# EDAPINENUT/CBGBench

Hardware: NVIDIA H100
Metric: ligands/sec sampled (1000-step denoise, batch 64) (higher is better)
Workload: dtype f32

## Files before the change

cbgbench_b200/csrc/cbg_tc.cuh:

```cuda
#pragma once
#include <cuda_fp16.h>
#include "cbg_common.cuh"

namespace cbg_tc {

__device__ __forceinline__ uint32_t smem_u32(const void* p) { return (uint32_t)__cvta_generic_to_shared(p); }

__device__ __forceinline__ void mbar_init(uint32_t bar, uint32_t count) {
  asm volatile("mbarrier.init.shared::cta.b64 [%0], %1;" ::"r"(bar), "r"(count));
}
__device__ __forceinline__ void mbar_expect_tx(uint32_t bar, uint32_t bytes) {
  asm volatile("mbarrier.arrive.expect_tx.shared::cta.b64 _, [%0], %1;" ::"r"(bar), "r"(bytes) : "memory");
}
__device__ __forceinline__ void mbar_arrive(uint32_t bar) {
  asm volatile("mbarrier.arrive.shared::cta.b64 _, [%0];" ::"r"(bar) : "memory");
}
__device__ __forceinline__ uint64_t global_timer_ns() {
  uint64_t t;
  asm volatile("mov.u64 %0, %%globaltimer;" : "=l"(t));
  return t;
}
__device__ __forceinline__ uint32_t mbar_try_wait(uint32_t bar, uint32_t parity) {
  uint32_t done;
  asm volatile(
      "{\n\t.reg .pred p;\n\t"
      "mbarrier.try_wait.parity.shared::cta.b64 p, [%1], %2, %3;\n\t"
      "selp.u32 %0, 1, 0, p;\n\t}"
      : "=r"(done)
      : "r"(bar), "r"(parity), "r"(100000u)
      : "memory");
  return done;
}
__device__ __forceinline__ void mbar_wait(uint32_t bar, uint32_t parity) {
  uint32_t spins = 0;
  uint64_t t0 = 0;
  while (!mbar_try_wait(bar, parity)) {
    if ((++spins & 1023u) == 0u) {
      const uint64_t t = global_timer_ns();
      if (t0 == 0) t0 = t;
      else if (t - t0 > 2000000000ull) __trap();
    }
  }
}
__device__ __forceinline__ void fence_mbar_init() { asm volatile("fence.mbarrier_init.release.cluster;" ::: "memory"); }
__device__ __forceinline__ void fence_proxy_async() { asm volatile("fence.proxy.async.shared::cta;" ::: "memory"); }

__device__ __forceinline__ void bulk_g2s(uint32_t dst, const void* src, uint32_t bytes, uint32_t bar) {
  asm volatile("cp.async.bulk.shared::cluster.global.mbarrier::complete_tx::bytes [%0], [%1], %2, [%3];" ::"r"(dst),
               "l"(src), "r"(bytes), "r"(bar)
               : "memory");
}
__device__ __forceinline__ void cp_async16(uint32_t dst, const void* src) {
  asm volatile("cp.async.cg.shared.global [%0], [%1], 16;" ::"r"(dst), "l"(src) : "memory");
}
__device__ __forceinline__ void cp_async_arrive(uint32_t bar) {
  asm volatile("cp.async.mbarrier.arrive.noinc.shared::cta.b64 [%0];" ::"r"(bar) : "memory");
}

__device__ __forceinline__ void pdl_launch_dependents() { asm volatile("griddepcontrol.launch_dependents;" ::: "memory"); }
__device__ __forceinline__ void pdl_wait() { asm volatile("griddepcontrol.wait;" ::: "memory"); }

__device__ __forceinline__ void wgmma_fence() { asm volatile("wgmma.fence.sync.aligned;" ::: "memory"); }
__device__ __forceinline__ void wgmma_commit() { asm volatile("wgmma.commit_group.sync.aligned;" ::: "memory"); }
__device__ __forceinline__ void wgmma_wait0() { asm volatile("wgmma.wait_group.sync.aligned 0;" ::: "memory"); }
template <int N>
__device__ __forceinline__ void wgmma_settle(float (&d)[N]) {
#pragma unroll
  for (int i = 0; i < N; ++i) asm volatile("" : "+f"(d[i])::"memory");
}
__device__ __forceinline__ void warpgroup_sync(int wg) { asm volatile("bar.sync %0, 128;" ::"r"(1 + wg) : "memory"); }
__device__ __forceinline__ uint64_t smem_desc(uint32_t saddr, uint32_t lbo_bytes, uint32_t sbo_bytes) {
  return (uint64_t)((saddr & 0x3FFFFu) >> 4) | ((uint64_t)(lbo_bytes >> 4) << 16) | ((uint64_t)(sbo_bytes >> 4) << 32);
}
__device__ __forceinline__ void wgmma_f16_ss(float (&d)[64], uint64_t adesc, uint64_t bdesc, uint32_t accumulate) {
  asm volatile(
      "{\n\t.reg .pred p;\n\t"
      "setp.ne.b32 p, %66, 0;\n\t"
      "wgmma.mma_async.sync.aligned.m64n128k16.f32.f16.f16 "
      "{%0, %1, %2, %3, %4, %5, %6, %7, %8, %9, %10, %11, %12, %13, %14, %15, %16, %17, %18, %19, %20, %21, %22, %23, %24, %25, %26, %27, %28, %29, %30, %31, %32, %33, %34, %35, %36, %37, %38, %39, %40, %41, %42, %43, %44, %45, %46, %47, %48, %49, %50, %51, %52, %53, %54, %55, %56, %57, %58, %59, %60, %61, %62, %63}, "
      "%64, %65, p, 1, 1, 0, 0;\n\t}"
      : "+f"(d[0]), "+f"(d[1]), "+f"(d[2]), "+f"(d[3]), "+f"(d[4]), "+f"(d[5]), "+f"(d[6]), "+f"(d[7]),
        "+f"(d[8]), "+f"(d[9]), "+f"(d[10]), "+f"(d[11]), "+f"(d[12]), "+f"(d[13]), "+f"(d[14]), "+f"(d[15]),
        "+f"(d[16]), "+f"(d[17]), "+f"(d[18]), "+f"(d[19]), "+f"(d[20]), "+f"(d[21]), "+f"(d[22]), "+f"(d[23]),
        "+f"(d[24]), "+f"(d[25]), "+f"(d[26]), "+f"(d[27]), "+f"(d[28]), "+f"(d[29]), "+f"(d[30]), "+f"(d[31]),
        "+f"(d[32]), "+f"(d[33]), "+f"(d[34]), "+f"(d[35]), "+f"(d[36]), "+f"(d[37]), "+f"(d[38]), "+f"(d[39]),
        "+f"(d[40]), "+f"(d[41]), "+f"(d[42]), "+f"(d[43]), "+f"(d[44]), "+f"(d[45]), "+f"(d[46]), "+f"(d[47]),
        "+f"(d[48]), "+f"(d[49]), "+f"(d[50]), "+f"(d[51]), "+f"(d[52]), "+f"(d[53]), "+f"(d[54]), "+f"(d[55]),
        "+f"(d[56]), "+f"(d[57]), "+f"(d[58]), "+f"(d[59]), "+f"(d[60]), "+f"(d[61]), "+f"(d[62]), "+f"(d[63])
      : "l"(adesc), "l"(bdesc), "r"(accumulate));
}
__device__ __forceinline__ void wgmma_f16_ss_first(float (&d)[64], uint64_t adesc, uint64_t bdesc) {
  asm volatile(
      "{\n\t.reg .pred p;\n\t"
      "setp.ne.b32 p, %66, 0;\n\t"
      "wgmma.mma_async.sync.aligned.m64n128k16.f32.f16.f16 "
      "{%0, %1, %2, %3, %4, %5, %6, %7, %8, %9, %10, %11, %12, %13, %14, %15, %16, %17, %18, %19, %20, %21, %22, %23, %24, %25, %26, %27, %28, %29, %30, %31, %32, %33, %34, %35, %36, %37, %38, %39, %40, %41, %42, %43, %44, %45, %46, %47, %48, %49, %50, %51, %52, %53, %54, %55, %56, %57, %58, %59, %60, %61, %62, %63}, "
      "%64, %65, p, 1, 1, 0, 0;\n\t}"
      : "=f"(d[0]), "=f"(d[1]), "=f"(d[2]), "=f"(d[3]), "=f"(d[4]), "=f"(d[5]), "=f"(d[6]), "=f"(d[7]),
        "=f"(d[8]), "=f"(d[9]), "=f"(d[10]), "=f"(d[11]), "=f"(d[12]), "=f"(d[13]), "=f"(d[14]), "=f"(d[15]),
        "=f"(d[16]), "=f"(d[17]), "=f"(d[18]), "=f"(d[19]), "=f"(d[20]), "=f"(d[21]), "=f"(d[22]), "=f"(d[23]),
        "=f"(d[24]), "=f"(d[25]), "=f"(d[26]), "=f"(d[27]), "=f"(d[28]), "=f"(d[29]), "=f"(d[30]), "=f"(d[31]),
        "=f"(d[32]), "=f"(d[33]), "=f"(d[34]), "=f"(d[35]), "=f"(d[36]), "=f"(d[37]), "=f"(d[38]), "=f"(d[39]),
        "=f"(d[40]), "=f"(d[41]), "=f"(d[42]), "=f"(d[43]), "=f"(d[44]), "=f"(d[45]), "=f"(d[46]), "=f"(d[47]),
        "=f"(d[48]), "=f"(d[49]), "=f"(d[50]), "=f"(d[51]), "=f"(d[52]), "=f"(d[53]), "=f"(d[54]), "=f"(d[55]),
        "=f"(d[56]), "=f"(d[57]), "=f"(d[58]), "=f"(d[59]), "=f"(d[60]), "=f"(d[61]), "=f"(d[62]), "=f"(d[63])
      : "l"(adesc), "l"(bdesc), "r"(0u));
}
__device__ __forceinline__ void wgmma_f16_rs(float (&d)[64], const uint32_t (&a)[4], uint64_t bdesc, uint32_t accumulate) {
  asm volatile(
      "{\n\t.reg .pred p;\n\t"
      "setp.ne.b32 p, %69, 0;\n\t"
      "wgmma.mma_async.sync.aligned.m64n128k16.f32.f16.f16 "
      "{%0, %1, %2, %3, %4, %5, %6, %7, %8, %9, %10, %11, %12, %13, %14, %15, %16, %17, %18, %19, %20, %21, %22, %23, %24, %25, %26, %27, %28, %29, %30, %31, %32, %33, %34, %35, %36, %37, %38, %39, %40, %41, %42, %43, %44, %45, %46, %47, %48, %49, %50, %51, %52, %53, %54, %55, %56, %57, %58, %59, %60, %61, %62, %63}, "
      "{%64, %65, %66, %67}, %68, p, 1, 1, 0;\n\t}"
      : "+f"(d[0]), "+f"(d[1]), "+f"(d[2]), "+f"(d[3]), "+f"(d[4]), "+f"(d[5]), "+f"(d[6]), "+f"(d[7]),
        "+f"(d[8]), "+f"(d[9]), "+f"(d[10]), "+f"(d[11]), "+f"(d[12]), "+f"(d[13]), "+f"(d[14]), "+f"(d[15]),
        "+f"(d[16]), "+f"(d[17]), "+f"(d[18]), "+f"(d[19]), "+f"(d[20]), "+f"(d[21]), "+f"(d[22]), "+f"(d[23]),
        "+f"(d[24]), "+f"(d[25]), "+f"(d[26]), "+f"(d[27]), "+f"(d[28]), "+f"(d[29]), "+f"(d[30]), "+f"(d[31]),
        "+f"(d[32]), "+f"(d[33]), "+f"(d[34]), "+f"(d[35]), "+f"(d[36]), "+f"(d[37]), "+f"(d[38]), "+f"(d[39]),
        "+f"(d[40]), "+f"(d[41]), "+f"(d[42]), "+f"(d[43]), "+f"(d[44]), "+f"(d[45]), "+f"(d[46]), "+f"(d[47]),
        "+f"(d[48]), "+f"(d[49]), "+f"(d[50]), "+f"(d[51]), "+f"(d[52]), "+f"(d[53]), "+f"(d[54]), "+f"(d[55]),
        "+f"(d[56]), "+f"(d[57]), "+f"(d[58]), "+f"(d[59]), "+f"(d[60]), "+f"(d[61]), "+f"(d[62]), "+f"(d[63])
      : "r"(a[0]), "r"(a[1]), "r"(a[2]), "r"(a[3]), "l"(bdesc), "r"(accumulate));
}
__device__ __forceinline__ void wgmma_f16_rs_n16(float (&d)[8], const uint32_t (&a)[4], uint64_t bdesc, uint32_t accumulate) {
  asm volatile(
      "{\n\t.reg .pred p;\n\t"
      "setp.ne.b32 p, %13, 0;\n\t"
      "wgmma.mma_async.sync.aligned.m64n16k16.f32.f16.f16 "
      "{%0, %1, %2, %3, %4, %5, %6, %7}, "
      "{%8, %9, %10, %11}, %12, p, 1, 1, 0;\n\t}"
      : "+f"(d[0]), "+f"(d[1]), "+f"(d[2]), "+f"(d[3]), "+f"(d[4]), "+f"(d[5]), "+f"(d[6]), "+f"(d[7])
      : "r"(a[0]), "r"(a[1]), "r"(a[2]), "r"(a[3]), "l"(bdesc), "r"(accumulate));
}
__device__ __forceinline__ void wgmma_tf32_ss(float (&d)[64], uint64_t adesc, uint64_t bdesc, uint32_t accumulate) {
  asm volatile(
      "{\n\t.reg .pred p;\n\t"
      "setp.ne.b32 p, %66, 0;\n\t"
      "wgmma.mma_async.sync.aligned.m64n128k8.f32.tf32.tf32 "
      "{%0, %1, %2, %3, %4, %5, %6, %7, %8, %9, %10, %11, %12, %13, %14, %15, %16, %17, %18, %19, %20, %21, %22, %23, %24, %25, %26, %27, %28, %29, %30, %31, %32, %33, %34, %35, %36, %37, %38, %39, %40, %41, %42, %43, %44, %45, %46, %47, %48, %49, %50, %51, %52, %53, %54, %55, %56, %57, %58, %59, %60, %61, %62, %63}, "
      "%64, %65, p, 1, 1;\n\t}"
      : "+f"(d[0]), "+f"(d[1]), "+f"(d[2]), "+f"(d[3]), "+f"(d[4]), "+f"(d[5]), "+f"(d[6]), "+f"(d[7]),
        "+f"(d[8]), "+f"(d[9]), "+f"(d[10]), "+f"(d[11]), "+f"(d[12]), "+f"(d[13]), "+f"(d[14]), "+f"(d[15]),
        "+f"(d[16]), "+f"(d[17]), "+f"(d[18]), "+f"(d[19]), "+f"(d[20]), "+f"(d[21]), "+f"(d[22]), "+f"(d[23]),
        "+f"(d[24]), "+f"(d[25]), "+f"(d[26]), "+f"(d[27]), "+f"(d[28]), "+f"(d[29]), "+f"(d[30]), "+f"(d[31]),
        "+f"(d[32]), "+f"(d[33]), "+f"(d[34]), "+f"(d[35]), "+f"(d[36]), "+f"(d[37]), "+f"(d[38]), "+f"(d[39]),
        "+f"(d[40]), "+f"(d[41]), "+f"(d[42]), "+f"(d[43]), "+f"(d[44]), "+f"(d[45]), "+f"(d[46]), "+f"(d[47]),
        "+f"(d[48]), "+f"(d[49]), "+f"(d[50]), "+f"(d[51]), "+f"(d[52]), "+f"(d[53]), "+f"(d[54]), "+f"(d[55]),
        "+f"(d[56]), "+f"(d[57]), "+f"(d[58]), "+f"(d[59]), "+f"(d[60]), "+f"(d[61]), "+f"(d[62]), "+f"(d[63])
      : "l"(adesc), "l"(bdesc), "r"(accumulate));
}

__device__ __forceinline__ void cluster_sync_all() {
  asm volatile("barrier.cluster.arrive.release.aligned;\n\tbarrier.cluster.wait.acquire.aligned;" ::: "memory");
}
__device__ __forceinline__ uint32_t cluster_rank() {
  uint32_t r;
  asm volatile("mov.u32 %0, %%cluster_ctarank;" : "=r"(r));
  return r;
}
__device__ __forceinline__ void bulk_g2s_mcast(uint32_t dst, const void* src, uint32_t bytes, uint32_t bar, uint16_t mask) {
  asm volatile(
      "cp.async.bulk.shared::cluster.global.mbarrier::complete_tx::bytes.multicast::cluster [%0], [%1], %2, [%3], %4;" ::"r"(dst),
      "l"(src), "r"(bytes), "r"(bar), "h"(mask)
      : "memory");
}
__device__ __forceinline__ void mbar_arrive_cluster(uint32_t bar, uint32_t rank) {
  asm volatile(
      "{\n\t.reg .b32 ra;\n\t"
      "mapa.shared::cluster.u32 ra, %0, %1;\n\t"
      "mbarrier.arrive.release.cluster.shared::cluster.b64 _, [ra];\n\t}" ::"r"(bar), "r"(rank)
      : "memory");
}

__device__ __forceinline__ uint32_t pack_h2(float lo_elem, float hi_elem) {
  const __half2 h = __floats2half2_rn(lo_elem, hi_elem);
  return *reinterpret_cast<const uint32_t*>(&h);
}
__device__ __forceinline__ void split_pair(float x0, float x1, uint32_t& hi, uint32_t& lo) {
  const __half2 h = __floats2half2_rn(x0, x1);
  const float2 hf = __half22float2(h);
  hi = *reinterpret_cast<const uint32_t*>(&h);
  lo = pack_h2(x0 - hf.x, x1 - hf.y);
}
__device__ __forceinline__ void split_pair_relu(float x0, float x1, uint32_t& hi, uint32_t& lo) {
  const float h0 = __uint_as_float(__float_as_uint(x0) & 0xffffe000u);
  const float h1 = __uint_as_float(__float_as_uint(x1) & 0xffffe000u);
  const float2 l = fadd2(make_float2(x0, x1), make_float2(-h0, -h1));
  asm("cvt.rn.relu.f16x2.f32 %0, %1, %2;" : "=r"(hi) : "f"(h1), "f"(h0));
  asm("cvt.rn.relu.f16x2.f32 %0, %1, %2;" : "=r"(lo) : "f"(l.y), "f"(l.x));
}

}
```

cbgbench_b200/csrc/x2h_tc.cu:

```cuda
#include <math.h>
#include <stdlib.h>
#include <string.h>
#include <type_traits>
#include "cbg_kernels.cuh"
#include "cbg_tc.cuh"

using namespace cbg_tc;

namespace {

constexpr long long kOffKW1 = cbg_layout::layer_offset(CBG_LF_X2H_K_TCW1);
constexpr long long kOffKWg = cbg_layout::layer_offset(CBG_LF_X2H_K_TCWG);
constexpr long long kOffVW1 = cbg_layout::layer_offset(CBG_LF_X2H_V_TCW1);
constexpr long long kOffVWg = cbg_layout::layer_offset(CBG_LF_X2H_V_TCWG);
constexpr long long kOffKLn = cbg_layout::layer_offset(CBG_LF_X2H_K_LN);
constexpr long long kOffVLn = cbg_layout::layer_offset(CBG_LF_X2H_V_LN);
constexpr long long kOffVB1 = cbg_layout::layer_offset(CBG_LF_X2H_V_B1);
constexpr long long kOffRbf = cbg_layout::layer_offset(CBG_LF_X2H_K_RBF);
constexpr long long kOffXKW1 = cbg_layout::layer_offset(CBG_LF_H2X_K_TCW1);
constexpr long long kOffXKWg = cbg_layout::layer_offset(CBG_LF_H2X_K_TCWG);
constexpr long long kOffXVW1 = cbg_layout::layer_offset(CBG_LF_H2X_V_TCW1);
constexpr long long kOffXVWg = cbg_layout::layer_offset(CBG_LF_H2X_V_TCWG);
constexpr long long kOffXKLn = cbg_layout::layer_offset(CBG_LF_H2X_K_LN);
constexpr long long kOffXVLn = cbg_layout::layer_offset(CBG_LF_H2X_V_LN);
constexpr long long kOffXVB1 = cbg_layout::layer_offset(CBG_LF_H2X_V_B1);
constexpr long long kOffXRbf = cbg_layout::layer_offset(CBG_LF_H2X_RBF);

enum { MODE_K = 0, MODE_V = 1, MODE_XV = 2 };
struct TcWeights {
  const float* w1;
  const float* wg;
  const float* ln;
  const float* b1;
  const float* rbf;
};

constexpr float kInvPre = 1.f / 16384.f;
constexpr uint32_t kHalfTypeOne = 0x6400u;
constexpr float kScaleA = 64.f;
constexpr float kInvOut = 1.f / 4096.f;

constexpr int KG = 96;
constexpr int KG_LO = 80;
constexpr uint32_t W1_IMG = 128 * 128 * 2;
constexpr uint32_t W1X_IMG = 16 * 128 * 2;
constexpr uint32_t WG_IMG = 128 * KG * 2;
constexpr uint32_t G_IMG = 64 * KG * 2;
constexpr uint32_t W1_SBO = (128 / 8) * 128, WG_SBO = (KG / 8) * 128, LBO = 128;
constexpr uint32_t SM_W1 = 0;
constexpr uint32_t SM_WG = SM_W1 + 2 * W1_IMG;
constexpr uint32_t SM_G = SM_WG + 2 * WG_IMG;
constexpr uint32_t SM_LN = SM_G + 4 * G_IMG;
constexpr uint32_t SM_B1 = SM_LN + 1024;
constexpr uint32_t SM_RBF = SM_B1 + 512;
constexpr uint32_t SM_EPI = SM_RBF + 128;
constexpr uint32_t P_ROW = CBG_H * 4;
constexpr uint32_t STG_WARP = P_ROW + 8 * (P_ROW + 32);
constexpr uint32_t SM_BAR = SM_EPI + 4 * 32 * 17 * 4;
constexpr uint32_t SM_STG = SM_BAR + 128;
constexpr uint32_t sm_total(bool stage) { return stage ? SM_STG + 8 * STG_WARP : SM_STG; }
static_assert(sm_total(true) <= 232448, "shared memory budget");
static_assert(SM_STG % 16 == 0 && STG_WARP % 16 == 0, "bulk-copy destinations are 16-byte aligned");
enum { B_WFULL = 0 , B_W1FULL , B_STG  };
__host__ __device__ constexpr uint32_t stg_pj_row(int r) { return P_ROW + (P_ROW + 32u) * (uint32_t)r; }

__device__ __forceinline__ int list_len(const EdgeArgs& p) {
  int n = p.n_nodes;
  if (p.n_nodes_dev) { const int nd = *p.n_nodes_dev; n = nd < n ? nd : n; }
  return n;
}
__device__ __forceinline__ int node_of(const EdgeArgs& p, int n, int n_list) {
  const int nc = n < n_list ? n : n_list - 1;
  return p.node_idx ? p.node_idx[nc] : nc;
}
__device__ __forceinline__ float quad_sum(float v) {
  v += __shfl_xor_sync(CBG_FULL, v, 1);
  return v + __shfl_xor_sync(CBG_FULL, v, 2);
}
__device__ __forceinline__ float rows_sum(float v) {
  v += __shfl_xor_sync(CBG_FULL, v, 4);
  v += __shfl_xor_sync(CBG_FULL, v, 8);
  return v + __shfl_xor_sync(CBG_FULL, v, 16);
}
template <int IB, int LB, int LEVELS, int N, int LIVE = N>
__device__ __forceinline__ void reduce_scatter(float (&a)[N], int lane) {
  static_assert((LIVE >> LEVELS) << LEVELS == LIVE && (LIVE >> LEVELS) >= (1 << IB), "reduce_scatter shape");
  const bool up = (lane >> LB) & 1;
#pragma unroll
  for (int o = 0; o < LIVE / 2; ++o) {
    const int i0 = ((o >> IB) << (IB + 1)) | (o & ((1 << IB) - 1)), i1 = i0 | (1 << IB);
    const float give = up ? a[i0] : a[i1];
    const float keep = up ? a[i1] : a[i0];
    a[o] = keep + __shfl_xor_sync(CBG_FULL, give, 1 << LB);
  }
  if constexpr (LEVELS > 1) reduce_scatter<IB, LB + 1, LEVELS - 1, N, LIVE / 2>(a, lane);
}
__device__ __forceinline__ float2 ldg2(const float* p) { return __ldg(reinterpret_cast<const float2*>(p)); }

#define TC_STAMP(k, ev)                                                                                  \
  do {                                                                                                   \
    if (p.trace != nullptr && blockIdx.x == 0 && tid == 0 && (k) < p.trace_tiles) p.trace[(k) * 16 + (ev)] = clock64(); \
  } while (0)

template <int MODE, bool STAGE>
__global__ void __launch_bounds__(256, 1) x2h_tc_kernel(EdgeArgs p, TcWeights W) {
  constexpr bool IS_V = MODE == MODE_V, IS_XV = MODE == MODE_XV;
  extern __shared__ __align__(1024) uint8_t smem[];
  const int tid = threadIdx.x, warp = tid >> 5, lane = tid & 31;
  const uint32_t sbase = smem_u32(smem);
  constexpr uint32_t W1B = IS_XV ? W1X_IMG : W1_IMG;
  const uint32_t bars = sbase + SM_BAR;
  auto bar = [&](int i) { return bars + 8u * (uint32_t)i; };

  pdl_launch_dependents();
#define TC_STAMP_CTA(ev) do { if (p.trace != nullptr && blockIdx.x == 0 && tid == 0) p.trace[p.trace_tiles * 16 + (ev)] = clock64(); } while (0)
  TC_STAMP_CTA(0);
  if (tid == 32) {
    mbar_init(bar(B_WFULL), 1);
    mbar_init(bar(B_W1FULL), 1);
    if constexpr (STAGE) {
      for (int w = 0; w < 8; ++w) mbar_init(bar(B_STG + w), 1);
    }
    fence_mbar_init();
    mbar_expect_tx(bar(B_WFULL), 2 * WG_IMG);
    mbar_expect_tx(bar(B_W1FULL), 2 * W1B);
    const uint32_t rot = blockIdx.x & 3u;
#pragma unroll
    for (uint32_t i = 0; i < 4; ++i) {
      const uint32_t pc = (i + rot) & 3u, nb = (2 * WG_IMG) / 4;
      bulk_g2s(sbase + SM_WG + pc * nb, reinterpret_cast<const uint8_t*>(W.wg) + pc * nb, nb, bar(B_WFULL));
    }
#pragma unroll
    for (uint32_t i = 0; i < 4; ++i) {
      const uint32_t pc = (i + rot) & 3u, nb = (2 * W1B) / 4;
      bulk_g2s(sbase + SM_W1 + pc * nb, reinterpret_cast<const uint8_t*>(W.w1) + pc * nb, nb, bar(B_W1FULL));
    }
  }
  {
    float* s_ln = reinterpret_cast<float*>(smem + SM_LN);
    float* s_b1 = reinterpret_cast<float*>(smem + SM_B1);
    s_ln[tid] = W.ln[tid] * kScaleA;
    if (tid < 128) s_b1[tid] = (IS_V || (IS_XV && tid < CBG_HEADS)) ? W.b1[tid] : 0.f;
    else if (tid < 128 + 24) reinterpret_cast<float*>(smem + SM_RBF)[tid - 128] = W.rbf[tid - 128];
  }
  pdl_wait();
  const int n_list = list_len(p);
  const int n_tiles = (n_list + 3) >> 2;
  const bool has_work = (int)blockIdx.x < n_tiles;
  const int n_my = has_work ? (n_tiles - 1 - (int)blockIdx.x) / (int)gridDim.x + 1 : 0;
  auto tile_node = [&](int kk, int slot) { return node_of(p, 4 * ((int)blockIdx.x + kk * (int)gridDim.x) + slot, n_list); };
  __syncthreads();
  TC_STAMP_CTA(1);
  mbar_wait(bar(B_WFULL), 0u);
  mbar_wait(bar(B_W1FULL), 0u);

  const int wg = warp >> 2, w4 = warp & 3, qg = lane >> 2, qt = lane & 3;
  const int g_row = tid & 63, g_part = (tid >> 6) & 1;
  const int g_slot = 2 * wg + (g_row >> 5);
  const int slot = 2 * wg + (w4 >> 1), wp = w4 & 1, e0 = 16 * wp + qg;
  const float* rbf = reinterpret_cast<const float*>(smem + SM_RBF);
  const float c2 = rbf[20] * 1.4426950408889634f;
  const float* s_ln = reinterpret_cast<const float*>(smem + SM_LN);
  const float* s_b1 = reinterpret_cast<const float*>(smem + SM_B1);
  float* s_epi = reinterpret_cast<float*>(smem + SM_EPI);
  const float* pj_plane = MODE != MODE_K ? p.pj_v : p.pj_k;
  const float* pi_plane = MODE != MODE_K ? p.pi_v : p.pi_k;
  const uint32_t g_base = sbase + SM_G + (uint32_t)wg * 2u * G_IMG;
  const uint64_t dg_hi = smem_desc(g_base, LBO, WG_SBO), dg_lo = smem_desc(g_base + G_IMG, LBO, WG_SBO);
  const uint64_t dw_hi = smem_desc(sbase + SM_WG, LBO, WG_SBO), dw_lo = smem_desc(sbase + SM_WG + WG_IMG, LBO, WG_SBO);
  const uint64_t d1_hi = smem_desc(sbase + SM_W1, LBO, W1_SBO), d1_lo = smem_desc(sbase + SM_W1 + W1B, LBO, W1_SBO);

  auto load_idx = [&](int kk, int& gi, int& gjn, int& ti, int& tj0, int& tj1) {
    gi = tile_node(kk, g_slot);
    gjn = p.nbr[(size_t)gi * CBG_KMAX + (g_row & 31)];
    ti = tile_node(kk, slot);
    const size_t eoff = (size_t)ti * CBG_KMAX + e0;
    tj0 = p.nbr[eoff];
    tj1 = p.nbr[eoff + 8];
  };
  auto build_g = [&](const float4 xi, const float4 xj) {
    const float rx = xi.x - xj.x, ry = xi.y - xj.y, rz = xi.z - xj.z;
    const float d = sqrtf(__fmaf_rn(rz, rz, __fmaf_rn(ry, ry, __fmul_rn(rx, rx))));
    const int fi = node_flags(xi), fj = node_flags(xj);
    const int t_e = ((fj & 1) ? 0 : 2) + ((fi & 1) ? 0 : 1);
    uint32_t gv[10];
#pragma unroll
    for (int mp = 0; mp < 10; ++mp) {
      const float u0 = d - rbf[2 * mp], u1 = d - rbf[2 * mp + 1];
      float g0, g1;
      asm("ex2.approx.ftz.f32 %0, %1;" : "=f"(g0) : "f"(fmaf(c2 * u0, u0, 10.f)));
      asm("ex2.approx.ftz.f32 %0, %1;" : "=f"(g1) : "f"(fmaf(c2 * u1, u1, 10.f)));
      uint32_t hi, lo;
      split_pair(g0, g1, hi, lo);
      gv[mp] = g_part ? lo : hi;
    }
    uint8_t* grow = smem + SM_G + (uint32_t)(2 * wg + g_part) * G_IMG + (uint32_t)(g_row >> 3) * WG_SBO + (uint32_t)(g_row & 7) * 16u;
#pragma unroll
    for (int c = 0; c < KG_LO / 8; ++c) {
      uint4 w;
      w.x = (t_e == (4 * c) / 10) ? gv[(4 * c) % 10] : 0u;
      w.y = (t_e == (4 * c + 1) / 10) ? gv[(4 * c + 1) % 10] : 0u;
      w.z = (t_e == (4 * c + 2) / 10) ? gv[(4 * c + 2) % 10] : 0u;
      w.w = (t_e == (4 * c + 3) / 10) ? gv[(4 * c + 3) % 10] : 0u;
      *reinterpret_cast<uint4*>(grow + 128u * c) = w;
    }
    if (g_part == 0) {
      uint4 w = make_uint4(0u, 0u, 0u, 0u);
      w.x = (t_e == 0) ? kHalfTypeOne : ((t_e == 1) ? (kHalfTypeOne << 16) : 0u);
      w.y = (t_e == 2) ? kHalfTypeOne : ((t_e == 3) ? (kHalfTypeOne << 16) : 0u);
      *reinterpret_cast<uint4*>(grow + 128u * 10) = w;
      *reinterpret_cast<uint4*>(grow + 128u * 11) = make_uint4(0u, 0u, 0u, 0u);
    }
  };
  auto issue_mma1 = [&](float (&d)[64]) {
    wgmma_fence();
#pragma unroll
    for (int ks = 0; ks < KG_LO / 16; ++ks) {
      if (ks == 0) wgmma_f16_ss_first(d, dg_lo, dw_hi);
      else wgmma_f16_ss(d, dg_lo + 16u * ks, dw_hi + 16u * ks, 1u);
    }
#pragma unroll
    for (int ks = 0; ks < KG / 16; ++ks) wgmma_f16_ss(d, dg_hi + 16u * ks, dw_lo + 16u * ks, 1u);
#pragma unroll
    for (int ks = 0; ks < KG / 16; ++ks) wgmma_f16_ss(d, dg_hi + 16u * ks, dw_hi + 16u * ks, 1u);
    wgmma_commit();
    wgmma_settle(d);
  };
  auto gather_p = [&](float (&v)[64], int j, int ti, int tj0, int tj1) {
    const float2 a = ldg2(pi_plane + (size_t)ti * CBG_H + 2 * qt + 8 * j);
    const float2 b0 = ldg2(pj_plane + (size_t)(tj0 >= 0 ? tj0 : ti) * CBG_H + 2 * qt + 8 * j);
    const float2 b1 = ldg2(pj_plane + (size_t)(tj1 >= 0 ? tj1 : ti) * CBG_H + 2 * qt + 8 * j);
    v[4 * j] = a.x + b0.x; v[4 * j + 1] = a.y + b0.y; v[4 * j + 2] = a.x + b1.x; v[4 * j + 3] = a.y + b1.y;
  };
  const uint32_t stg = sbase + SM_STG + (uint32_t)warp * STG_WARP;
  const uint8_t* s_stg = smem + SM_STG + (uint32_t)warp * STG_WARP;
  auto stage_rows = [&](int sti, int stj0) {
    __syncwarp();
    if (lane == 0) mbar_expect_tx(bar(B_STG + warp), 9 * P_ROW);
    if (qt == 0) bulk_g2s(stg + stg_pj_row(qg), pj_plane + (size_t)(stj0 >= 0 ? stj0 : sti) * CBG_H, P_ROW, bar(B_STG + warp));
    else if (lane == 1) bulk_g2s(stg, pi_plane + (size_t)sti * CBG_H, P_ROW, bar(B_STG + warp));
  };
  auto gather_pj1 = [&](float (&b)[32], int sti, int stj1) {
    const float* r = pj_plane + (size_t)(stj1 >= 0 ? stj1 : sti) * CBG_H + 2 * qt;
#pragma unroll
    for (int j = 0; j < 16; ++j) { const float2 t = ldg2(r + 8 * j); b[2 * j] = t.x; b[2 * j + 1] = t.y; }
  };

  float d[64];
  float v[64];
  float pj1[32];
  int ti = 0, tj0 = 0, tj1 = 0;
  int ngi = 0, ngjn = 0, nti = 0, ntj0 = 0, ntj1 = 0;
  if (n_my > 0) {
    int gi, gjn;
    load_idx(0, gi, gjn, ti, tj0, tj1);
    if constexpr (STAGE) {
      stage_rows(ti, tj0);
      gather_pj1(pj1, ti, tj1);
    }
    build_g(p.x4[gi], p.x4[gjn >= 0 ? gjn : gi]);
    fence_proxy_async();
    warpgroup_sync(wg);
    issue_mma1(d);
    if constexpr (!STAGE) {
#pragma unroll
      for (int j = 0; j < 16; ++j) gather_p(v, j, ti, tj0, tj1);
    }
  }
  auto tile = [&](const int k, auto more_c) {
    constexpr bool more = decltype(more_c)::value;
    if constexpr (more) load_idx(k + 1, ngi, ngjn, nti, ntj0, ntj1);
    wgmma_wait0();
    wgmma_settle(d);
    TC_STAMP(k, 0);
    const int n = 4 * ((int)blockIdx.x + k * (int)gridDim.x) + slot;
    const bool live = n < n_list;
    const int i = ti;
    const int w_row = p.w_compact ? (n < n_list ? n : n_list - 1) : i;
    uint32_t a_hi[8][4], a_lo[8][4];
    {
      float q0 = 0.f, q1 = 0.f;
      if constexpr (STAGE) {
        mbar_wait(bar(B_STG + warp), (uint32_t)k & 1u);
        const float* s_pi = reinterpret_cast<const float*>(s_stg) + 2 * qt;
        const float* s_pj = reinterpret_cast<const float*>(s_stg + stg_pj_row(qg)) + 2 * qt;
#pragma unroll
        for (int j = 0; j < 16; ++j) {
          const float2 a = *reinterpret_cast<const float2*>(s_pi + 8 * j);
          const float2 b0 = *reinterpret_cast<const float2*>(s_pj + 8 * j);
          v[4 * j] = a.x + b0.x; v[4 * j + 1] = a.y + b0.y; v[4 * j + 2] = a.x + pj1[2 * j]; v[4 * j + 3] = a.y + pj1[2 * j + 1];
        }
      }
#pragma unroll
      for (int j = 0; j < 16; ++j) {
        v[4 * j] = fmaf(d[4 * j], kInvPre, v[4 * j]);
        v[4 * j + 1] = fmaf(d[4 * j + 1], kInvPre, v[4 * j + 1]);
        v[4 * j + 2] = fmaf(d[4 * j + 2], kInvPre, v[4 * j + 2]);
        v[4 * j + 3] = fmaf(d[4 * j + 3], kInvPre, v[4 * j + 3]);
        q0 = fmaf(v[4 * j], v[4 * j], q0); q0 = fmaf(v[4 * j + 1], v[4 * j + 1], q0);
        q1 = fmaf(v[4 * j + 2], v[4 * j + 2], q1); q1 = fmaf(v[4 * j + 3], v[4 * j + 3], q1);
      }
      float rs[2];
#pragma unroll
      for (int h = 0; h < 2; ++h) {
        const float var = quad_sum(h ? q1 : q0) * (1.f / 128.f) + 1e-5f;
        const float r = rsqrtf(var);
        rs[h] = r * (1.5f - 0.5f * var * r * r);
      }
#pragma unroll
      for (int j = 0; j < 16; ++j) {
        const float2 ga = *reinterpret_cast<const float2*>(s_ln + 8 * j + 2 * qt);
        const float2 be = *reinterpret_cast<const float2*>(s_ln + 128 + 8 * j + 2 * qt);
#pragma unroll
        for (int h = 0; h < 2; ++h) {
          const float y0 = fmaf(v[4 * j + 2 * h] * rs[h], ga.x, be.x), y1 = fmaf(v[4 * j + 2 * h + 1] * rs[h], ga.y, be.y);
          split_pair_relu(y0, y1, a_hi[j >> 1][2 * (j & 1) + h], a_lo[j >> 1][2 * (j & 1) + h]);
        }
      }
    }
    auto issue_mma2 = [&](auto& o) {
      wgmma_fence();
#pragma unroll
      for (int ks = 0; ks < 8; ++ks) {
        if constexpr (IS_XV) wgmma_f16_rs_n16(o, a_lo[ks], d1_hi + 16u * ks, ks > 0 ? 1u : 0u);
        else wgmma_f16_rs(o, a_lo[ks], d1_hi + 16u * ks, ks > 0 ? 1u : 0u);
      }
#pragma unroll
      for (int ks = 0; ks < 8; ++ks) {
        if constexpr (IS_XV) wgmma_f16_rs_n16(o, a_hi[ks], d1_lo + 16u * ks, 1u);
        else wgmma_f16_rs(o, a_hi[ks], d1_lo + 16u * ks, 1u);
      }
#pragma unroll
      for (int ks = 0; ks < 8; ++ks) {
        if constexpr (IS_XV) wgmma_f16_rs_n16(o, a_hi[ks], d1_hi + 16u * ks, 1u);
        else wgmma_f16_rs(o, a_hi[ks], d1_hi + 16u * ks, 1u);
      }
      wgmma_commit();
      wgmma_settle(o);
      TC_STAMP(k, 1);
    };
    auto advance = [&](auto& o) {
      if constexpr (more && STAGE) {
        stage_rows(nti, ntj0);
        gather_pj1(pj1, nti, ntj1);
      }
      if constexpr (more) {
        const float4 xi = p.x4[ngi], xj = p.x4[ngjn >= 0 ? ngjn : ngi];
        warpgroup_sync(wg);
        build_g(xi, xj);
        fence_proxy_async();
      } else {
        warpgroup_sync(wg);
      }
      wgmma_wait0();
      wgmma_settle(o);
      TC_STAMP(k, 2);
      if constexpr (more) {
        warpgroup_sync(wg);
        issue_mma1(d);
        TC_STAMP(k, 3);
      }
    };
    auto gather_next = [&](int j) { if constexpr (more && !STAGE) gather_p(v, j, nti, ntj0, ntj1); };
    if constexpr (MODE == MODE_K) {
      float qv[32];
      {
        const float* qr = p.q + (size_t)i * CBG_H + 2 * qt;
#pragma unroll
        for (int j = 0; j < 16; ++j) { const float2 t = ldg2(qr + 8 * j); qv[2 * j] = t.x; qv[2 * j + 1] = t.y; }
      }
      const int hd = lane & 15, eh = 16 * (lane >> 4);
      float sc[8];
#pragma unroll
      for (int j = 0; j < 8; ++j) {
        const size_t eo = (size_t)i * CBG_KMAX + eh + 8 * wp + j;
        sc[j] = p.nbr[eo] >= 0 ? p.ew[eo] : 0.f;
      }
      float o[64];
      issue_mma2(o);
      advance(o);
      float* s_sm = s_epi + slot * (32 * 17);
#pragma unroll
      for (int m = 0; m < 4; ++m) {
        float lg[8];
#pragma unroll
        for (int jj = 0; jj < 4; ++jj) {
          const int j = 4 * m + jj;
          lg[2 * jj] = fmaf(o[4 * j + 1], qv[2 * j + 1], o[4 * j] * qv[2 * j]);
          lg[2 * jj + 1] = fmaf(o[4 * j + 3], qv[2 * j + 1], o[4 * j + 2] * qv[2 * j]);
          gather_next(j);
        }
        reduce_scatter<1, 0, 2>(lg, lane);
        s_sm[e0 * 17 + 4 * m + qt] = tj0 >= 0 ? lg[0] * kInvOut : -INFINITY;
        s_sm[(e0 + 8) * 17 + 4 * m + qt] = tj1 >= 0 ? lg[1] * kInvOut : -INFINITY;
      }
      warpgroup_sync(wg);
      {
        float l[16];
        float mx = -INFINITY;
#pragma unroll
        for (int j = 0; j < 16; ++j) { l[j] = s_sm[(eh + j) * 17 + hd]; mx = fmaxf(mx, l[j]); }
        mx = fmaxf(mx, __shfl_xor_sync(CBG_FULL, mx, 16));
        float sum = 0.f;
#pragma unroll
        for (int j = 0; j < 16; ++j) { l[j] = (mx == -INFINITY) ? 0.f : __expf(l[j] - mx); sum += l[j]; }
        sum += __shfl_xor_sync(CBG_FULL, sum, 16);
        const float inv = 1.f / ((sum > 0.f) ? sum : 1.f);
        if (live) {
          float* wo = p.w + ((size_t)w_row * CBG_KMAX + eh + 8 * wp) * CBG_HEADS + hd;
#pragma unroll
          for (int j = 0; j < 8; ++j) wo[j * CBG_HEADS] = (wp ? l[8 + j] : l[j]) * inv * sc[j];
        }
      }
    } else if constexpr (IS_V) {
      float wv[2][CBG_HEADS];
#pragma unroll
      for (int h = 0; h < 2; ++h) {
        const float* wi = p.w + ((size_t)w_row * CBG_KMAX + e0 + 8 * h) * CBG_HEADS;
#pragma unroll
        for (int j = 0; j < 4; ++j) {
          const float4 t = ld4(wi + 4 * j);
          wv[h][4 * j] = t.x; wv[h][4 * j + 1] = t.y; wv[h][4 * j + 2] = t.z; wv[h][4 * j + 3] = t.w;
        }
      }
      const int c = 2 * (32 * wp + lane);
      float2* hp = reinterpret_cast<float2*>(p.h + (size_t)i * CBG_H + c);
      const float2 hv = *hp;
      float o[64];
      issue_mma2(o);
      advance(o);
      float* s_vr = s_epi + (slot * 2 + wp) * CBG_H;
#pragma unroll
      for (int b = 0; b < 2; ++b) {
        float s[16];
#pragma unroll
        for (int jj = 0; jj < 8; ++jj) {
          const int j = 8 * b + jj;
          const float2 b1 = *reinterpret_cast<const float2*>(s_b1 + 8 * j + 2 * qt);
          s[2 * jj] = fmaf(fmaf(o[4 * j + 2], kInvOut, b1.x), wv[1][j], fmaf(o[4 * j], kInvOut, b1.x) * wv[0][j]);
          s[2 * jj + 1] = fmaf(fmaf(o[4 * j + 3], kInvOut, b1.y), wv[1][j], fmaf(o[4 * j + 1], kInvOut, b1.y) * wv[0][j]);
          gather_next(j);
        }
        reduce_scatter<1, 2, 3>(s, lane);
        *reinterpret_cast<float2*>(s_vr + 64 * b + 8 * qg + 2 * qt) = make_float2(s[0], s[1]);
      }
      warpgroup_sync(wg);
      if (live) {
        const float* s0 = s_epi + (slot * 2) * CBG_H + c;
        *hp = make_float2(hv.x + (s0[0] + s0[CBG_H]), hv.y + (s0[1] + s0[CBG_H + 1]));
      }
    } else {
      float2 wx[2][2];
      float rel[2][3];
      {
        const float4 xi = p.x4[i];
#pragma unroll
        for (int h = 0; h < 2; ++h) {
          const float* wi = p.w + ((size_t)w_row * CBG_KMAX + e0 + 8 * h) * CBG_HEADS + 2 * qt;
          wx[h][0] = *reinterpret_cast<const float2*>(wi);
          wx[h][1] = *reinterpret_cast<const float2*>(wi + 8);
          const int jn = h ? tj1 : tj0;
          const float4 xj = p.x4[jn >= 0 ? jn : i];
          rel[h][0] = xi.x - xj.x; rel[h][1] = xi.y - xj.y; rel[h][2] = xi.z - xj.z;
        }
      }
      float o[8];
      issue_mma2(o);
      advance(o);
#pragma unroll
      for (int j = 0; j < 16; ++j) gather_next(j);
      float se[2];
#pragma unroll
      for (int h = 0; h < 2; ++h) {
        float acc = 0.f;
#pragma unroll
        for (int j = 0; j < 2; ++j) {
          const float2 b1 = *reinterpret_cast<const float2*>(s_b1 + 8 * j + 2 * qt);
          acc = fmaf(fmaf(o[4 * j + 2 * h], kInvOut, b1.x), wx[h][j].x, acc);
          acc = fmaf(fmaf(o[4 * j + 2 * h + 1], kInvOut, b1.y), wx[h][j].y, acc);
        }
        se[h] = quad_sum(acc);
      }
      float* s_dx = s_epi + (slot * 2 + wp) * 4;
#pragma unroll
      for (int c = 0; c < 3; ++c) {
        const float a = rows_sum(fmaf(se[1], rel[1][c], se[0] * rel[0][c]));
        if (lane == 0) s_dx[c] = a;
      }
      warpgroup_sync(wg);
      if (live && wp == 0 && lane == 0) {
        const float* s0 = s_epi + slot * 8;
        st4(p.dx + 4 * (size_t)n, make_float4((s0[0] + s0[4]) * (1.f / 16.f), (s0[1] + s0[5]) * (1.f / 16.f), (s0[2] + s0[6]) * (1.f / 16.f), 0.f));
      }
    }
    TC_STAMP(k, 4);
    ti = nti; tj0 = ntj0; tj1 = ntj1;
  };
  for (int k = 0; k + 1 < n_my; ++k) tile(k, std::true_type{});
  if (n_my > 0) tile(n_my - 1, std::false_type{});
  TC_STAMP_CTA(2);
}

__global__ void __launch_bounds__(128, 1) wgmma_selftest_kernel(const __half* a, const __half* b, float* d, int a_from_smem) {
  extern __shared__ __align__(1024) uint8_t smem[];
  const int tid = threadIdx.x, warp = tid >> 5, lane = tid & 31, qg = lane >> 2, qt = lane & 3;
  constexpr uint32_t SBO = (32 / 8) * 128;
  const uint32_t sbase = smem_u32(smem);
  const uint32_t sb_b = sbase, sb_a = sbase + 128 * 32 * 2;
  for (int e = tid; e < 128 * 32; e += 128) {
    const int r = e >> 5, kk = e & 31;
    const uint32_t off = (uint32_t)(r >> 3) * SBO + (uint32_t)(kk >> 3) * 128u + (uint32_t)(r & 7) * 16u + (uint32_t)(kk & 7) * 2u;
    *reinterpret_cast<__half*>(smem + off) = b[e];
    *reinterpret_cast<__half*>(smem + 128 * 32 * 2 + off) = a[e];
  }
  fence_proxy_async();
  __syncthreads();
#pragma unroll 1
  for (int half = 0; half < 2; ++half) {
    const int r0 = 64 * half + 16 * warp + qg;
    float acc[64];
    uint32_t af[2][4];
#pragma unroll
    for (int ks = 0; ks < 2; ++ks) {
      af[ks][0] = *reinterpret_cast<const uint32_t*>(a + (size_t)r0 * 32 + 16 * ks + 2 * qt);
      af[ks][1] = *reinterpret_cast<const uint32_t*>(a + (size_t)(r0 + 8) * 32 + 16 * ks + 2 * qt);
      af[ks][2] = *reinterpret_cast<const uint32_t*>(a + (size_t)r0 * 32 + 16 * ks + 8 + 2 * qt);
      af[ks][3] = *reinterpret_cast<const uint32_t*>(a + (size_t)(r0 + 8) * 32 + 16 * ks + 8 + 2 * qt);
    }
    wgmma_fence();
#pragma unroll
    for (int ks = 0; ks < 2; ++ks) {
      if (a_from_smem) wgmma_f16_ss(acc, smem_desc(sb_a + (uint32_t)(8 * half) * SBO + 256u * ks, 128, SBO), smem_desc(sb_b + 256u * ks, 128, SBO), ks > 0);
      else wgmma_f16_rs(acc, af[ks], smem_desc(sb_b + 256u * ks, 128, SBO), ks > 0);
    }
    wgmma_commit();
    wgmma_wait0();
    wgmma_settle(acc);
#pragma unroll
    for (int j = 0; j < 16; ++j) {
      *reinterpret_cast<float2*>(d + (size_t)r0 * 128 + 8 * j + 2 * qt) = make_float2(acc[4 * j], acc[4 * j + 1]);
      *reinterpret_cast<float2*>(d + (size_t)(r0 + 8) * 128 + 8 * j + 2 * qt) = make_float2(acc[4 * j + 2], acc[4 * j + 3]);
    }
  }
}

int g_tc_sms = 0;
bool g_tc_stage = true;
long long* g_tc_trace = nullptr;
int g_tc_trace_tiles = 0;

template <int MODE>
void launch_tc(int grid, cudaStream_t st, const EdgeArgs& a, const TcWeights& w) {
  if constexpr (MODE != MODE_V) {
    if (g_tc_stage) {
      cbg_launch_pdl(x2h_tc_kernel<MODE, true>, dim3(grid), dim3(256), sm_total(true), st, a, w);
      return;
    }
  }
  cbg_launch_pdl(x2h_tc_kernel<MODE, false>, dim3(grid), dim3(256), sm_total(false), st, a, w);
}

int tc_init() {
  static bool done_dev[CBG_MAX_DEVICES] = {};
  bool& done = cbg_dev_flag(done_dev);
  if (done) return 0;
  int dev = 0;
  CBG_CUDA_OK(cudaGetDevice(&dev));
  CBG_CUDA_OK(cudaDeviceGetAttribute(&g_tc_sms, cudaDevAttrMultiProcessorCount, dev));
  if (const char* e = getenv("CBG_X2H_STAGE")) g_tc_stage = strcmp(e, "0") != 0;
#define TC_ATTR(MODE, STAGE) CBG_CUDA_OK(cudaFuncSetAttribute(x2h_tc_kernel<MODE, STAGE>, cudaFuncAttributeMaxDynamicSharedMemorySize, (int)sm_total(STAGE)))
  TC_ATTR(MODE_K, true); TC_ATTR(MODE_XV, true);
  TC_ATTR(MODE_K, false); TC_ATTR(MODE_V, false); TC_ATTR(MODE_XV, false);
#undef TC_ATTR
  done = true;
  return 0;
}

}

int cbg_launch_x2h_tc(const EdgeArgs& a, cudaStream_t st) {
  if (a.n_nodes <= 0) return 0;
  if (int rc = tc_init()) return rc;
  const int tiles = (a.n_nodes + 3) / 4;
  const int grid = tiles < g_tc_sms ? tiles : g_tc_sms;
  EdgeArgs ak = a;
  ak.w_compact = 0;
  EdgeArgs av = a;
  av.w_compact = 0;
  if (g_tc_trace_tiles >= 0) { ak.trace = g_tc_trace; ak.trace_tiles = g_tc_trace_tiles; }
  else { av.trace = g_tc_trace; av.trace_tiles = -g_tc_trace_tiles; }
  g_tc_trace = nullptr;
  const float* L = a.layer;
  const TcWeights wk{L + kOffKW1, L + kOffKWg, L + kOffKLn, nullptr, L + kOffRbf};
  const TcWeights wv{L + kOffVW1, L + kOffVWg, L + kOffVLn, L + kOffVB1, L + kOffRbf};
  CBG_PROF_BEGIN(CBG_K_X2H_K, st);
  launch_tc<MODE_K>(grid, st, ak, wk);
  CBG_LAUNCHED(CBG_K_X2H_K, st);
  CBG_PROF_BEGIN(CBG_K_X2H_V, st);
  launch_tc<MODE_V>(grid, st, av, wv);
  CBG_LAUNCHED(CBG_K_X2H_V, st);
  return 0;
}

int cbg_launch_h2x_tc(const EdgeArgs& a, cudaStream_t st) {
  if (a.n_nodes <= 0) return 0;
  if (int rc = tc_init()) return rc;
  if (a.node_idx == nullptr || a.w == nullptr || a.dx == nullptr) { cbg_set_error("h2x_tc: node list, w and dx buffers are required"); return 1; }
  const int tiles = (a.n_nodes + 3) / 4;
  const int grid = tiles < g_tc_sms ? tiles : g_tc_sms;
  EdgeArgs ax = a;
  ax.w_compact = 1; ax.trace = nullptr; ax.trace_tiles = 0;
  const float* L = a.layer;
  const TcWeights wk{L + kOffXKW1, L + kOffXKWg, L + kOffXKLn, nullptr, L + kOffXRbf};
  const TcWeights wv{L + kOffXVW1, L + kOffXVWg, L + kOffXVLn, L + kOffXVB1, L + kOffXRbf};
  CBG_PROF_BEGIN(CBG_K_H2X, st);
  launch_tc<MODE_K>(grid, st, ax, wk);
  CBG_LAUNCHED(CBG_K_H2X, st);
  CBG_PROF_BEGIN(CBG_K_H2X, st);
  launch_tc<MODE_XV>(grid, st, ax, wv);
  CBG_LAUNCHED(CBG_K_H2X, st);
  return 0;
}

void cbg_x2h_tc_set_trace(long long* buf, int max_tiles) { g_tc_trace = buf; g_tc_trace_tiles = buf ? max_tiles : 0; }

int cbg_launch_umma_selftest(const void* a, const void* b, float* d, int a_from_smem, cudaStream_t st) {
  const int smem_bytes = 2 * 128 * 32 * 2;
  wgmma_selftest_kernel<<<1, 128, smem_bytes, st>>>((const __half*)a, (const __half*)b, d, a_from_smem);
  CBG_CUDA_OK(cudaGetLastError());
  return 0;
}
```

Measured before the change: 14.41.

## Skip zero K-chunks in first MMA when warpgroup rows share ligand class

After: 14.57 (median of 6 runs). +1.1%, better.

```diff
diff --git a/cbgbench_b200/csrc/cbg_tc.cuh b/cbgbench_b200/csrc/cbg_tc.cuh
--- a/cbgbench_b200/csrc/cbg_tc.cuh
+++ b/cbgbench_b200/csrc/cbg_tc.cuh
@@ -69,6 +69,17 @@
   for (int i = 0; i < N; ++i) asm volatile("" : "+f"(d[i])::"memory");
 }
 __device__ __forceinline__ void warpgroup_sync(int wg) { asm volatile("bar.sync %0, 128;" ::"r"(1 + wg) : "memory"); }
+__device__ __forceinline__ uint32_t warpgroup_sync_count(int wg, int pred) {
+  uint32_t n;
+  asm volatile(
+      "{\n\t.reg .pred p;\n\t"
+      "setp.ne.b32 p, %2, 0;\n\t"
+      "bar.red.popc.u32 %0, %1, 128, p;\n\t}"
+      : "=r"(n)
+      : "r"(1 + wg), "r"(pred)
+      : "memory");
+  return n;
+}
 __device__ __forceinline__ uint64_t smem_desc(uint32_t saddr, uint32_t lbo_bytes, uint32_t sbo_bytes) {
   return (uint64_t)((saddr & 0x3FFFFu) >> 4) | ((uint64_t)(lbo_bytes >> 4) << 16) | ((uint64_t)(sbo_bytes >> 4) << 32);
 }
diff --git a/cbgbench_b200/csrc/x2h_tc.cu b/cbgbench_b200/csrc/x2h_tc.cu
--- a/cbgbench_b200/csrc/x2h_tc.cu
+++ b/cbgbench_b200/csrc/x2h_tc.cu
@@ -47,6 +47,8 @@
 constexpr uint32_t WG_IMG = 128 * KG * 2;
 constexpr uint32_t G_IMG = 64 * KG * 2;
 constexpr uint32_t W1_SBO = (128 / 8) * 128, WG_SBO = (KG / 8) * 128, LBO = 128;
+constexpr uint64_t CM = LBO >> 4;
+constexpr uint64_t WIN_LBO3 = (uint64_t)((3 * LBO - LBO) >> 4) << 16;
 constexpr uint32_t SM_W1 = 0;
 constexpr uint32_t SM_WG = SM_W1 + 2 * W1_IMG;
 constexpr uint32_t SM_G = SM_WG + 2 * WG_IMG;
@@ -103,8 +105,9 @@
   } while (0)
 
 template <int MODE, bool STAGE>
-__global__ void __launch_bounds__(256, 1) x2h_tc_kernel(EdgeArgs p, TcWeights W) {
+__global__ void __launch_bounds__(256, 1) x2h_tc_kernel(EdgeArgs p, TcWeights W, int window) {
   constexpr bool IS_V = MODE == MODE_V, IS_XV = MODE == MODE_XV;
+  constexpr bool WINDOWS = MODE != MODE_K;
   extern __shared__ __align__(1024) uint8_t smem[];
   const int tid = threadIdx.x, warp = tid >> 5, lane = tid & 31;
   const uint32_t sbase = smem_u32(smem);
@@ -212,18 +215,46 @@
       *reinterpret_cast<uint4*>(grow + 128u * 11) = make_uint4(0u, 0u, 0u, 0u);
     }
   };
-  auto issue_mma1 = [&](float (&d)[64]) {
-    wgmma_fence();
-#pragma unroll
-    for (int ks = 0; ks < KG_LO / 16; ++ks) {
-      if (ks == 0) wgmma_f16_ss_first(d, dg_lo, dw_hi);
-      else wgmma_f16_ss(d, dg_lo + 16u * ks, dw_hi + 16u * ks, 1u);
-    }
-#pragma unroll
-    for (int ks = 0; ks < KG / 16; ++ks) wgmma_f16_ss(d, dg_hi + 16u * ks, dw_lo + 16u * ks, 1u);
-#pragma unroll
-    for (int ks = 0; ks < KG / 16; ++ks) wgmma_f16_ss(d, dg_hi + 16u * ks, dw_hi + 16u * ks, 1u);
-    wgmma_commit();
+  auto g_handoff = [&](int lig) {
+    if constexpr (!WINDOWS) {
+      warpgroup_sync(wg);
+      return -1;
+    }
+    const uint32_t n_lig = warpgroup_sync_count(wg, lig);
+    const bool mixed = n_lig != 0u && n_lig != 128u;
+    if (p.trace != nullptr && (tid & 127) == 0) {
+      unsigned long long* cnt = reinterpret_cast<unsigned long long*>(p.trace + p.trace_tiles * 16);
+      atomicAdd(cnt + 3, 1ull);
+      if (mixed) atomicAdd(cnt + 4, 1ull);
+    }
+    return __shfl_sync(CBG_FULL, (mixed || !window) ? -1 : (n_lig != 0u ? 0 : 1), 0);
+  };
+  auto issue_mma1 = [&](float (&d)[64], int cls) {
+    if (cls >= 0) {
+      wgmma_fence();
+      const uint64_t o = 2 * CM * (uint64_t)cls;
+      const uint64_t win[4] = {o, 2 * CM + o + WIN_LBO3, 6 * CM + o, 10 * CM};
+      wgmma_f16_ss_first(d, dg_lo + win[0], dw_hi + win[0]);
+#pragma unroll
+      for (int w = 1; w < 3; ++w) wgmma_f16_ss(d, dg_lo + win[w], dw_hi + win[w], 1u);
+#pragma unroll
+      for (int w = 0; w < 4; ++w) wgmma_f16_ss(d, dg_hi + win[w], dw_lo + win[w], 1u);
+#pragma unroll
+      for (int w = 0; w < 4; ++w) wgmma_f16_ss(d, dg_hi + win[w], dw_hi + win[w], 1u);
+      wgmma_commit();
+    } else {
+      wgmma_fence();
+#pragma unroll
+      for (int ks = 0; ks < KG_LO / 16; ++ks) {
+        if (ks == 0) wgmma_f16_ss_first(d, dg_lo, dw_hi);
+        else wgmma_f16_ss(d, dg_lo + 16u * ks, dw_hi + 16u * ks, 1u);
+      }
+#pragma unroll
+      for (int ks = 0; ks < KG / 16; ++ks) wgmma_f16_ss(d, dg_hi + 16u * ks, dw_lo + 16u * ks, 1u);
+#pragma unroll
+      for (int ks = 0; ks < KG / 16; ++ks) wgmma_f16_ss(d, dg_hi + 16u * ks, dw_hi + 16u * ks, 1u);
+      wgmma_commit();
+    }
     wgmma_settle(d);
   };
   auto gather_p = [&](float (&v)[64], int j, int ti, int tj0, int tj1) {
@@ -258,10 +289,10 @@
       stage_rows(ti, tj0);
       gather_pj1(pj1, ti, tj1);
     }
-    build_g(p.x4[gi], p.x4[gjn >= 0 ? gjn : gi]);
+    const float4 xi = p.x4[gi];
+    build_g(xi, p.x4[gjn >= 0 ? gjn : gi]);
     fence_proxy_async();
-    warpgroup_sync(wg);
-    issue_mma1(d);
+    issue_mma1(d, g_handoff(node_flags(xi) & 1));
     if constexpr (!STAGE) {
 #pragma unroll
       for (int j = 0; j < 16; ++j) gather_p(v, j, ti, tj0, tj1);
@@ -344,8 +375,10 @@
         stage_rows(nti, ntj0);
         gather_pj1(pj1, nti, ntj1);
       }
+      [[maybe_unused]] int lig = 0;
       if constexpr (more) {
         const float4 xi = p.x4[ngi], xj = p.x4[ngjn >= 0 ? ngjn : ngi];
+        lig = node_flags(xi) & 1;
         warpgroup_sync(wg);
         build_g(xi, xj);
         fence_proxy_async();
@@ -356,8 +389,7 @@
       wgmma_settle(o);
       TC_STAMP(k, 2);
       if constexpr (more) {
-        warpgroup_sync(wg);
-        issue_mma1(d);
+        issue_mma1(d, g_handoff(lig));
         TC_STAMP(k, 3);
       }
     };
@@ -546,6 +578,7 @@
 
 int g_tc_sms = 0;
 bool g_tc_stage = true;
+int g_tc_window = 1;
 long long* g_tc_trace = nullptr;
 int g_tc_trace_tiles = 0;
 
@@ -553,11 +586,11 @@
 void launch_tc(int grid, cudaStream_t st, const EdgeArgs& a, const TcWeights& w) {
   if constexpr (MODE != MODE_V) {
     if (g_tc_stage) {
-      cbg_launch_pdl(x2h_tc_kernel<MODE, true>, dim3(grid), dim3(256), sm_total(true), st, a, w);
+      cbg_launch_pdl(x2h_tc_kernel<MODE, true>, dim3(grid), dim3(256), sm_total(true), st, a, w, g_tc_window);
       return;
     }
   }
-  cbg_launch_pdl(x2h_tc_kernel<MODE, false>, dim3(grid), dim3(256), sm_total(false), st, a, w);
+  cbg_launch_pdl(x2h_tc_kernel<MODE, false>, dim3(grid), dim3(256), sm_total(false), st, a, w, g_tc_window);
 }
 
 int tc_init() {
@@ -568,6 +601,7 @@
   CBG_CUDA_OK(cudaGetDevice(&dev));
   CBG_CUDA_OK(cudaDeviceGetAttribute(&g_tc_sms, cudaDevAttrMultiProcessorCount, dev));
   if (const char* e = getenv("CBG_X2H_STAGE")) g_tc_stage = strcmp(e, "0") != 0;
+  if (const char* e = getenv("CBG_X2H_MMA1_WINDOW")) g_tc_window = strcmp(e, "0") != 0;
 #define TC_ATTR(MODE, STAGE) CBG_CUDA_OK(cudaFuncSetAttribute(x2h_tc_kernel<MODE, STAGE>, cudaFuncAttributeMaxDynamicSharedMemorySize, (int)sm_total(STAGE)))
   TC_ATTR(MODE_K, true); TC_ATTR(MODE_XV, true);
   TC_ATTR(MODE_K, false); TC_ATTR(MODE_V, false); TC_ATTR(MODE_XV, false);
```
